# microsoft/fadtk

Measured on NVIDIA H100. Metric: audio_seconds_embedded_per_second, higher is better.
Workload: dtype f16

## Files before the change

fadtk_b200/csrc/fadtk_b200.cu:

```cuda
#include "../../include/fadtk_b200.h"

#include <cuda.h>
#include <cuda_runtime.h>
#include <cuda_fp16.h>
#include <cxxabi.h>
#include <algorithm>
#include <cmath>
#include <cstdio>
#include <cstdlib>
#include <cstring>
#include <memory>
#include <set>
#include <string>
#include <type_traits>
#include <utility>
#include <vector>

#include "conv_gemm.cuh"
#include "frontend.cuh"
#include "stats.cuh"
#include "frechet.cuh"
#include "clap.cuh"
#include "resample.cuh"
#include "whisper.cuh"
// ... 200 lines not shown
                 cudaLaunchAttribute* attrs, unsigned n_attrs, Args&&... args) {
    if (grid.x == 0 || grid.y == 0 || grid.z == 0) return 0;
    cudaLaunchConfig_t cfg = {};
    cfg.gridDim = grid;
    cfg.blockDim = block;
    cfg.dynamicSmemBytes = smem;
    cfg.stream = st;
    cfg.attrs = attrs;
    cfg.numAttrs = n_attrs;
    cudaError_t e = cudaLaunchKernelEx(&cfg, kernel, std::forward<Args>(args)...);
    const cudaError_t last = cudaGetLastError();
    if (e == cudaSuccess) e = last;
    if (e != cudaSuccess) return fail(kernel_name((const void*)kernel) + ": " + cudaGetErrorString(e));
    h->launches++;
    return 0;
}
template <typename... Params, typename... Args>
int launch(fad_handle* h, void (*kernel)(Params...), dim3 grid, dim3 block, size_t smem, cudaStream_t st, Args&&... args) {
    return launch_attrs(h, kernel, grid, block, smem, st, nullptr, 0, std::forward<Args>(args)...);
}

template <int WMODE> struct Gemm {
    static constexpr int kStages = WMODE ? 3 : 4;
    static constexpr uint32_t kSmem = fad::conv_gemm_smem_bytes<128, kStages, WMODE>();
    static_assert(kSmem <= 227 * 1024, "over the per-CTA shared-memory limit");
    static constexpr auto kernel = fad::conv_gemm_kernel<128, kStages, WMODE>;
};

cudaLaunchAttribute cta_pair() {
    cudaLaunchAttribute attr = {};
    attr.id = cudaLaunchAttributeClusterDimension;
    attr.val.clusterDim.x = fad::kClusterCtas; attr.val.clusterDim.y = 1; attr.val.clusterDim.z = 1;
    return attr;
}

template <int WMODE>
int setup_gemm(fad_handle* h) {
    CK(cudaFuncSetAttribute(Gemm<WMODE>::kernel, cudaFuncAttributeMaxDynamicSharedMemorySize, (int)Gemm<WMODE>::kSmem));
    cudaLaunchAttribute attr = cta_pair();
    cudaLaunchConfig_t cfg = {};
    cfg.gridDim = dim3(fad::kClusterCtas * (unsigned)h->num_sms);
    cfg.blockDim = dim3(fad::kConvGemmThreads);
    cfg.dynamicSmemBytes = Gemm<WMODE>::kSmem;
    cfg.attrs = &attr;
    cfg.numAttrs = 1;
    CK(cudaOccupancyMaxActiveClusters(&h->gemm_clusters[WMODE], Gemm<WMODE>::kernel, &cfg));
    if (h->gemm_clusters[WMODE] <= 0) return fail("conv_gemm_kernel: no CTA pair fits on the device");
    return 0;
}

template <int WMODE>
int launch_conv_gemm(fad_handle* h, const CUtensorMap& mx, const CUtensorMap& mw, const fad::ConvGemmParams& p, cudaStream_t st) {
    const int units = (p.img_groups * p.tiles_h * p.tiles_w + 1) / 2 * p.n_tiles;
    cudaLaunchAttribute attr = cta_pair();
    return launch_attrs(h, Gemm<WMODE>::kernel, dim3(fad::kClusterCtas * (unsigned)std::min(units, h->gemm_clusters[WMODE])),
                        dim3(fad::kConvGemmThreads), Gemm<WMODE>::kSmem, st, &attr, 1, mx, mw, p);
}

int encode_layer_maps(const LayerGeom& g, const void* x, long long nb_dim, const void* w,
                      CUtensorMap* mx, CUtensorMap* mw, int a_cols = 0, long long a_row_stride = 0) {
    const uint64_t ac = a_cols > 0 ? (uint64_t)a_cols : (uint64_t)g.Cin;
    const uint64_t xd[4] = {ac, (uint64_t)g.W, (uint64_t)g.H, (uint64_t)nb_dim};
    uint64_t xs[3] = {ac * 2, (uint64_t)g.W * ac * 2, (uint64_t)g.H * g.W * ac * 2};
    if (a_row_stride > 0) xs[0] = xs[1] = xs[2] = (uint64_t)a_row_stride * 2;
    const uint32_t xb[4] = {64, (uint32_t)g.box_w, (uint32_t)g.box_h, (uint32_t)g.box_n};
    if (encode_f16_map(mx, x, 4, xd, xs, xb)) return 1;
    const uint64_t K = (uint64_t)g.taps * g.Cin;
    const uint64_t rows_mul = g.split_w ? 2 : 1;
    const uint64_t wd[2] = {K, (uint64_t)g.Cout * rows_mul};
    const uint64_t ws[1] = {K * 2};
    const uint32_t wb[2] = {64, (uint32_t)(g.n_tile * rows_mul / fad::kClusterCtas)};
    return encode_f16_map(mw, w, 2, wd, ws, wb);
}

int launch_attention_wgmma(fad_handle* h, const __half* qkv, long long n_clips, int S, int d, int heads, __half* out, cudaStream_t st) {
    if (heads * 64 != d) return fail("attention_wgmma: head dimension must be 64");
    CUtensorMap map;
    const uint64_t dims[3] = {(uint64_t)3 * d, (uint64_t)S, (uint64_t)n_clips};
    const uint64_t strides[2] = {(uint64_t)3 * d * 2, (uint64_t)S * 3 * d * 2};
    const uint32_t box[3] = {64, 128, 1};
    if (encode_f16_map(&map, qkv, 3, dims, strides, box)) return 1;
    fad::AttnParams p;
    p.S = S; p.d = d; p.heads = heads; p.out = out;
    return launch(h, fad::attention_wgmma_kernel, dim3((S + 127) / 128, heads, (unsigned)n_clips), fad::kAtThreads, fad::kAtSmem,
                  st, map, p);
}

int run_layer(fad_handle* h, const LayerGeom& g, const CUtensorMap& mx, const CUtensorMap& mw, const void* w,
              int NB, const float* bias, void* out, float* out_f32, cudaStream_t st,
              float* resid = nullptr, int resid_C = 0, int resid_res = 0, int resid_shift = 0, int n_valid = 0) {
    fad::ConvGemmParams p;
    p.taps = g.taps; p.cblks = g.Cin / 64;
    p.box_w = g.box_w; p.box_h = g.box_h; p.box_n = g.box_n;
    p.tiles_w = g.W / g.box_w; p.tiles_h = g.H / g.box_h;
    p.img_groups = (NB + g.box_n - 1) / g.box_n;
    p.n_tiles = g.Cout / g.n_tile;
    p.H = g.H; p.W = g.W; p.NB = NB; p.Cout = g.Cout;
    p.n_valid = n_valid > 0 ? n_valid : g.Cout;
    p.ld_out = p.n_valid;
    p.relu = g.relu; p.pool = g.pool;
    p.bias = bias; p.out = reinterpret_cast<__half*>(out); p.out_f32 = out_f32;
    p.resid = resid; p.resid_C = resid_C; p.resid_res = resid_res; p.resid_shift = resid_shift;
    p.lo_adds = g.split_w == 1 && h->zero_lo.count(w) == 0;
    if (g.split_w) return launch_conv_gemm<1>(h, mx, mw, p, st);
    return launch_conv_gemm<0>(h, mx, mw, p, st);
}

__global__ void wlo_absmax_kernel(const __half* __restrict__ w, long long n_tiles, long long K, unsigned int* __restrict__ out) {
    float m = 0.f;
    const long long total = n_tiles * 128 * K;
    for (long long e = blockIdx.x * (long long)blockDim.x + threadIdx.x; e < total; e += (long long)gridDim.x * blockDim.x) {
        const long long row = e / K, k = e - row * K;
        const long long t = row >> 7, j = row & 127;
        m = fmaxf(m, fabsf(__half2float(w[((t * 256 + 128 + j) * K) + k])));
    }
    for (int o = 16; o > 0; o >>= 1) m = fmaxf(m, __shfl_xor_sync(0xffffffffu, m, o));
    if ((threadIdx.x & 31) == 0) atomicMax(out, __float_as_uint(m));
}
int note_split_weights(fad_handle* h, const void* w, long long n_tiles, long long K, cudaStream_t st) {
    DeviceBuffer d_max;
    if (d_max.grow(4)) return 1;
    unsigned int mx = 0;
    const unsigned blocks = (unsigned)std::max<long long>(1, std::min<long long>((n_tiles * 128 * K + 255) / 256, (long long)h->num_sms * 16));
    CK(cudaMemsetAsync(d_max.get(), 0, 4, st));
    if (launch(h, wlo_absmax_kernel, blocks, 256, 0, st, reinterpret_cast<const __half*>(w), n_tiles, K, d_max.get<unsigned int>()))
        return 1;
    CK(cudaMemcpyAsync(&mx, d_max.get(), 4, cudaMemcpyDeviceToHost, st));
    CK(cudaStreamSynchronize(st));
    if (mx == 0) h->zero_lo.insert(w); else h->zero_lo.erase(w);
    return 0;
}

int upload_split(fad_handle* h, std::vector<DeviceBuffer>& mem, __half** dst, const void* src, size_t n, size_t k) {
    if (upload(mem, dst, src, 2 * n * k * 2)) return 1;
    return note_split_weights(h, *dst, (long long)(n / 128), (long long)k, 0);
}

struct VggLayer { int H, W, Cin, Cout, taps, relu, pool; };
const VggLayer kVgg[8] = {
    {48, 32, 64, 128, 9, 1, 1},
    {24, 16, 128, 256, 9, 1, 0},
    {24, 16, 256, 256, 9, 1, 1},
    {12, 8, 256, 512, 9, 1, 0},
    {12, 8, 512, 512, 9, 1, 1},
    {1, 1, 12288, 4096, 1, 1, 0},
    {1, 1, 4096, 4096, 1, 1, 0},
    {1, 1, 4096, 128, 1, 0, 0},
};
const size_t kActElems[8] = {48 * 32 * 64, 24 * 16 * 128, 24 * 16 * 256, 12 * 8 * 256,
                             12 * 8 * 512, 6 * 4 * 512, 4096, 4096};

struct VggState {
    std::vector<DeviceBuffer> mem;
    float *conv1_w = nullptr, *conv1_b = nullptr;
    __half* w[8] = {};
    float* b[8] = {};
    float* logmel = nullptr;
    __half* act[8] = {};
    CUtensorMap map_x[8], map_w[8];
    LayerGeom geom[8];
};

void build_frontend_tables(std::vector<double>& tw, std::vector<double>& hann,
                           std::vector<double>& melw, std::vector<int>& mstart, std::vector<int>& mcount) {
    const double PI = 3.14159265358979323846;
    tw.resize(512); hann.resize(fad::kWin);
    for (int k = 0; k < 256; ++k) {
        tw[2 * k] = std::cos(-2.0 * PI * k / 512.0);
        tw[2 * k + 1] = std::sin(-2.0 * PI * k / 512.0);
    }
    for (int n = 0; n < fad::kWin; ++n) hann[n] = 0.5 - 0.5 * std::cos(2.0 * PI / fad::kWin * n);
    auto mel = [](double f) { return 1127.0 * std::log(1.0 + f / 700.0); };
    std::vector<double> bins(fad::kBins), edges(fad::kMel + 2);
    for (int i = 0; i < fad::kBins; ++i) bins[i] = mel(8000.0 * i / (fad::kBins - 1));
    const double lo = mel(125.0), hi = mel(7500.0);
    for (int i = 0; i < fad::kMel + 2; ++i) edges[i] = lo + (hi - lo) * i / (fad::kMel + 1);
    melw.assign(fad::kMel * fad::kMelMaxTaps, 0.0);
    mstart.assign(fad::kMel, 0); mcount.assign(fad::kMel, 0);
    for (int b = 0; b < fad::kMel; ++b) {
        const double l = edges[b], c = edges[b + 1], u = edges[b + 2];
        int first = -1, cnt = 0;
        for (int i = 1; i < fad::kBins; ++i) {
            const double w = std::fmax(0.0, std::fmin((bins[i] - l) / (c - l), (u - bins[i]) / (u - c)));
            if (w > 0.0) {
                if (first < 0) first = i;
                const int off = i - first;
                if (off < fad::kMelMaxTaps) { melw[b * fad::kMelMaxTaps + off] = w; cnt = off + 1; }
            }
        }
        mstart[b] = first < 0 ? 0 : first;
        mcount[b] = cnt;
    }
}

size_t prof_begin(fad_handle* h, cudaStream_t st) {
    if (!h->prof_on) return 0;
    if (h->ev_used == h->ev_pool.size()) { cudaEvent_t e; cudaEventCreate(&e); h->ev_pool.push_back(e); }
    cudaEventRecord(h->ev_pool[h->ev_used], st);
    return h->ev_used++;
}
void prof_end(fad_handle* h, int cat, size_t e0, cudaStream_t st) {
    if (!h->prof_on) return;
    const size_t e1 = prof_begin(h, st);
    h->spans.push_back({cat, e0, e1});
}

template <typename In>
int launch_stats_dmma(fad_handle* h, const In* E, long long n_rows, int d, const __half* shift, double* acc, cudaStream_t st) {
    constexpr bool kProf = sizeof(In) == 2;
    if (d <= 0 || d % 64 != 0) return fail("d must be a positive multiple of 64");
    fad::StatsDmmaParams p;
    p.n_rows = n_rows; p.d = d; p.n_tiles = d / fad::kSdTile;
    p.n_pairs = p.n_tiles * (p.n_tiles + 1) / 2;
    const long long stages = (n_rows + fad::kSdRows - 1) / fad::kSdRows;
    long long want = (4LL * h->num_sms + p.n_pairs - 1) / p.n_pairs;
    if (want < 1) want = 1;
    long long per = (stages + want - 1) / want;
    if (per < 4) per = 4;
    p.n_splits = (int)((stages + per - 1) / per);
    p.rows_per_split = per * fad::kSdRows;
    p.shift = shift;
    const size_t jobs = (size_t)p.n_pairs * p.n_splits;
    if (h->ws_tiles.grow(jobs * fad::kSdTile * fad::kSdTile * 8)) return 1;
    if (h->ws_sums.grow((size_t)p.n_tiles * p.n_splits * fad::kSdTile * 8)) return 1;
    p.ws_tiles = h->ws_tiles.get<double>(); p.ws_sums = h->ws_sums.get<double>();
    size_t ev = kProf ? prof_begin(h, st) : 0;
    if (launch(h, fad::stats_dmma_kernel<In>, (unsigned)jobs, 256, 0, st, E, p)) return 1;
    if (kProf) { prof_end(h, FAD_PROF_STATS, ev, st); ev = prof_begin(h, st); }
    if (launch(h, fad::stats_dmma_reduce_kernel, dim3(p.n_pairs, fad::kSdTile * fad::kSdTile / 256), 256, 0, st, p, acc)) return 1;
    if (kProf) prof_end(h, FAD_PROF_STATS_REDUCE, ev, st);
    return 0;
}

}

extern "C" {

int fad_version(void) { return 1; }

int fad_profile_enable(fad_handle* h, int on) {
    if (!h) return fail("null handle");
    h->prof_on = on != 0;
    return 0;
}

int fad_profile_collect(fad_handle* h, double* ms_out, long long* count_out, int reset) {
    if (!h) return fail("null handle");
    CK(cudaSetDevice(h->device));
    CK(cudaDeviceSynchronize());
    for (const auto& sp : h->spans) {
        float ms = 0.f;
        if (cudaEventElapsedTime(&ms, h->ev_pool[sp.e0], h->ev_pool[sp.e1]) == cudaSuccess) {
            h->prof_ms[sp.cat] += ms; h->prof_count[sp.cat]++;
        }
    }
    h->spans.clear(); h->ev_used = 0;
    for (int i = 0; i < FAD_PROF_CATEGORIES; ++i) {
        if (ms_out) ms_out[i] = h->prof_ms[i];
        if (count_out) count_out[i] = h->prof_count[i];
        if (reset) { h->prof_ms[i] = 0.0; h->prof_count[i] = 0; }
    }
    return 0;
}
const char* fad_last_error(void) { return g_err.c_str(); }

int fad_create(int device, int max_examples, fad_handle** out) {
    if (!out) return fail("null out pointer");
    int count = 0;
    if (cudaGetDeviceCount(&count) != cudaSuccess || count == 0)
        return fail("no CUDA device: fadtk_b200 has no CPU fallback");
    if (device < 0 || device >= count) return fail("bad device index");
    CK(cudaSetDevice(device));
    cudaDeviceProp prop;
    CK(cudaGetDeviceProperties(&prop, device));
    if (prop.major != 9) return fail("fadtk_b200 kernels are built for sm_90a (Hopper H100) only");
    std::unique_ptr<fad_handle> h(new fad_handle());
    h->device = device;
    h->num_sms = prop.multiProcessorCount;
    h->max_examples = max_examples > 0 ? max_examples : 2048;

    std::vector<double> tw, hann, melw; std::vector<int> ms, mc;
    build_frontend_tables(tw, hann, melw, ms, mc);
    if (upload(h->mem, &h->d_twiddle, tw.data(), tw.size() * 8) || upload(h->mem, &h->d_hann, hann.data(), hann.size() * 8) ||
        upload(h->mem, &h->d_melw, melw.data(), melw.size() * 8) || upload(h->mem, &h->d_mel_start, ms.data(), ms.size() * 4) ||
        upload(h->mem, &h->d_mel_count, mc.data(), mc.size() * 4)) return 1;
    const auto smem = [](const void* kernel, size_t bytes) {
        return cudaFuncSetAttribute(kernel, cudaFuncAttributeMaxDynamicSharedMemorySize, (int)bytes);
    };
    CK(smem((const void*)fad::logmel_kernel<double>, fad::logmel_smem_bytes<double>()));
    CK(smem((const void*)fad::logmel_kernel<float>, fad::logmel_smem_bytes<float>()));
    CK(smem((const void*)fad::clap_logmel_kernel, fad::clap_logmel_smem_bytes()));
    CK(smem((const void*)fad::attention_wgmma_kernel, fad::kAtSmem));
    CK(smem((const void*)fad::clap_window_attention_kernel<24>, fad::att_smem_bytes(24, fad::kAttWarps, fad::kAttStages)));
    CK(smem((const void*)fad::clap_window_attention_kernel<32>, fad::att_smem_bytes(32, fad::kAttWarps, fad::kAttStages)));
    CK(smem((const void*)fad::kad_tile_kernel<0>, fad::kKadSmemBytes));
    CK(smem((const void*)fad::kad_tile_kernel<1>, fad::kKadSmemBytes));
    CK(smem((const void*)fad::kad_tile_kernel<2>, fad::kKadSmemBytes));
    CK(smem((const void*)fad::kad_perm_tile_kernel, fad::kPermSmemBytes));
    CK(smem((const void*)fad::prdc_tile_kernel<0>, fad::kPairSmemBytes));
    CK(smem((const void*)fad::prdc_tile_kernel<1>, fad::kPairSmemBytes));
    CK(smem((const void*)fad::prdc_tile_kernel<2>, fad::kPairSmemBytes));
    CK(smem((const void*)fad::prdc_tile_kernel<3>, fad::kPrdcSongSmemBytes));
    CK(smem((const void*)fad::prdc_tile_kernel<4>, fad::kPairSmemBytes));
    CK(smem((const void*)fad::prdc_tile_kernel<5>, fad::kPrdcNearestSmemBytes));
    CK(smem((const void*)fad::prdc_tile_kernel<6>, fad::kPairSmemBytes));
    if (setup_gemm<0>(h.get()) || setup_gemm<1>(h.get())) return 1;
    *out = h.release();
    return 0;
}

int fad_destroy(fad_handle* h) {
    if (!h) return 0;
    cudaSetDevice(h->device);
    fad_comm_destroy(h);
    delete h;
    return 0;
}

long long fad_launch_count(fad_handle* h) { return h ? h->launches : 0; }

int fad_vggish_load(fad_handle* h, const fad_vggish_weights* w) {
    if (!h || !w) return fail("null argument");
    const void* src[18] = {w->conv1_w_host, w->conv1_b_host,
                           w->conv_w_host[0], w->conv_w_host[1], w->conv_w_host[2], w->conv_w_host[3], w->conv_w_host[4],
                           w->fc_w_host[0], w->fc_w_host[1], w->fc_w_host[2],
                           w->conv_b_host[0], w->conv_b_host[1], w->conv_b_host[2], w->conv_b_host[3], w->conv_b_host[4],
                           w->fc_b_host[0], w->fc_b_host[1], w->fc_b_host[2]};
    if (check_tensors("fad_vggish_load", src, 18)) return 1;
    const void* const* wsrc = src + 2;
    const void* const* bsrc = src + 10;
    CK(cudaSetDevice(h->device));
    h->vgg.reset();
    auto vs = std::make_unique<VggState>();
    auto& m = vs->mem;
    if (upload(m, &vs->conv1_w, src[0], 64 * 9 * 4) || upload(m, &vs->conv1_b, src[1], 64 * 4)) return 1;
    for (int i = 0; i < 8; ++i) {
        const VggLayer& L = kVgg[i];
        const size_t mul = ((w->split_mask >> i) & 1) ? 2 : 1;
        if (upload(m, &vs->w[i], wsrc[i], mul * L.Cout * L.taps * L.Cin * 2) || upload(m, &vs->b[i], bsrc[i], (size_t)L.Cout * 4))
            return 1;
    }
    for (int i = 0; i < 8; ++i)
        if (((w->split_mask >> i) & 1) &&
            note_split_weights(h, vs->w[i], kVgg[i].Cout / 128, (long long)kVgg[i].taps * kVgg[i].Cin, 0)) return 1;
    const size_t B = (size_t)h->max_examples;
    if (alloc(m, &vs->logmel, B * 96 * 64 * 4)) return 1;
    for (int i = 0; i < 8; ++i)
        if (alloc(m, &vs->act[i], B * kActElems[i] * 2)) return 1;
    for (int i = 0; i < 8; ++i) {
        const VggLayer& L = kVgg[i];
        if (make_geom(vs->geom[i], L.H, L.W, L.Cin, L.Cout, L.taps, L.relu, L.pool, (w->split_mask >> i) & 1)) return 1;
        if (encode_layer_maps(vs->geom[i], vs->act[i], (long long)B, vs->w[i], &vs->map_x[i], &vs->map_w[i])) return 1;
    }
    h->vgg = std::move(vs);
    return 0;
}

long long fad_vggish_num_examples(long long n_samples) {
    if (n_samples < fad::kWin) return 0;
    const long long t = 1 + (n_samples - fad::kWin) / fad::kHop;
    if (t < fad::kExFrames) return 0;
    return 1 + (t - fad::kExFrames) / fad::kExFrames;
}

long long fad_vggish_plan(const long long* clip_offsets_host, long long n_clips,
                          long long* ex_start_host, long long capacity, long long* rows_per_clip_host) {
    long long n = 0;
    for (long long c = 0; c < n_clips; ++c) {
        const long long len = clip_offsets_host[c + 1] - clip_offsets_host[c];
        const long long k = fad_vggish_num_examples(len);
        if (rows_per_clip_host) rows_per_clip_host[c] = k;
        for (long long e = 0; e < k; ++e, ++n)
            if (ex_start_host && n < capacity)
                ex_start_host[n] = clip_offsets_host[c] + e * (long long)(fad::kExFrames * fad::kHop);
    }
    return n;
}

static int launch_logmel(fad_handle* h, const int16_t* pcm, const long long* ex_start, long long n,
                         float* out, int use_double, cudaStream_t st) {
    fad::FrontendTables tab{h->d_twiddle, h->d_hann, h->d_melw, h->d_mel_start, h->d_mel_count};
    const long long frames = n * fad::kExFrames;
    long long blocks = (frames + fad::kFeWarps - 1) / fad::kFeWarps;
    const long long cap = (long long)h->num_sms * 8;
    if (blocks > cap) blocks = cap;
    if (use_double)
        return launch(h, fad::logmel_kernel<double>, (int)blocks, fad::kFeWarps * 32, fad::logmel_smem_bytes<double>(), st,
                      pcm, ex_start, (int)n, tab, out);
    return launch(h, fad::logmel_kernel<float>, (int)blocks, fad::kFeWarps * 32, fad::logmel_smem_bytes<float>(), st,
                  pcm, ex_start, (int)n, tab, out);
}

int fad_vggish_logmel(fad_handle* h, const int16_t* pcm, const long long* ex_start,
                      long long n_examples, float* logmel_out, int use_double, void* stream) {
    if (!h) return fail("null handle");
    CK(cudaSetDevice(h->device));
    return launch_logmel(h, pcm, ex_start, n_examples, logmel_out, use_double, (cudaStream_t)stream);
}

int fad_vggish_forward(fad_handle* h, const int16_t* pcm, const long long* ex_start,
                       long long n_examples, void* emb_out_f16, void* stream) {
    if (!h) return fail("null handle");
    if (!h->vgg) return fail("fad_vggish_load has not been called");
    CK(cudaSetDevice(h->device));
    const VggState& vs = *h->vgg;
    cudaStream_t st = (cudaStream_t)stream;
    static const int fe_double = []() { const char* e = getenv("FADTK_FRONTEND_FP64"); return (e && e[0] == '1') ? 1 : 0; }();
    for (long long base = 0; base < n_examples; base += h->max_examples) {
        const int nb = (int)((n_examples - base) < h->max_examples ? (n_examples - base) : h->max_examples);
        size_t ev = prof_begin(h, st);
        if (launch_logmel(h, pcm, ex_start + base, nb, vs.logmel, fe_double, st)) return 1;
        prof_end(h, FAD_PROF_LOGMEL, ev, st);
        ev = prof_begin(h, st);
        if (launch(h, fad::conv1_kernel, dim3(6, nb), 256, 0, st, vs.logmel, vs.conv1_w, vs.conv1_b, vs.act[0])) return 1;
        prof_end(h, FAD_PROF_CONV1, ev, st);
        for (int i = 0; i < 8; ++i) {
            void* out = (i == 7) ? (void*)((__half*)emb_out_f16 + (size_t)base * 128) : (void*)vs.act[i + 1];
            ev = prof_begin(h, st);
            if (run_layer(h, vs.geom[i], vs.map_x[i], vs.map_w[i], vs.w[i], nb, vs.b[i], out, nullptr, st)) return 1;
            prof_end(h, FAD_PROF_LAYER0 + i, ev, st);
        }
    }
    return 0;
}

int fad_vggish_conv1(fad_handle* h, const float* logmel, long long n_examples, void* out_f16, void* stream) {
    if (!h) return fail("null handle");
    if (!h->vgg) return fail("fad_vggish_load has not been called");
    if (n_examples <= 0) return 0;
    CK(cudaSetDevice(h->device));
    return launch(h, fad::conv1_kernel, dim3(6, (unsigned)n_examples), 256, 0, (cudaStream_t)stream,
                  logmel, h->vgg->conv1_w, h->vgg->conv1_b, reinterpret_cast<__half*>(out_f16));
}

int fad_umma_layer(fad_handle* h, const void* x_f16, int NB, int H, int W, int Cin,
                   const void* w_f16, const float* bias, int Cout, int taps, int relu, int pool,
                   int split_w, void* out_f16, float* out_f32_or_null, void* stream) {
    if (!h) return fail("null handle");
    if (split_w != 0 && split_w != 1) return fail("fad_umma_layer: split_w must be 0 (fp16 weights) or 1 (fp16 hi/lo pair)");
    CK(cudaSetDevice(h->device));
    LayerGeom g;
    if (make_geom(g, H, W, Cin, Cout, taps, relu, pool, split_w)) return 1;
    if (pool && out_f32_or_null) return fail("fp32 copy is only available for un-pooled layers");
    if (g.split_w == 1 && note_split_weights(h, w_f16, Cout / 128, (long long)taps * Cin, (cudaStream_t)stream)) return 1;
    CUtensorMap mx, mw;
    if (encode_layer_maps(g, x_f16, NB, w_f16, &mx, &mw)) return 1;
    return run_layer(h, g, mx, mw, w_f16, NB, bias, out_f16, out_f32_or_null, (cudaStream_t)stream);
}

size_t fad_stats_acc_len(int d) { return 1 + 2 * (size_t)d + (size_t)d * d; }

int fad_stats_accumulate(fad_handle* h, const void* emb_f16, long long n_rows, int d,
                         const void* shift_f16, double* acc, int tensor_core, void* stream) {
    if (!h) return fail("null handle");
    if (tensor_core != 0 && tensor_core != 2) return fail("fad_stats_accumulate: tensor_core must be 0 (DMMA) or 2 (CUDA-core fp64)");
    if (n_rows <= 0) return 0;
    CK(cudaSetDevice(h->device));
    cudaStream_t st = (cudaStream_t)stream;
    const __half* E = reinterpret_cast<const __half*>(emb_f16);
    const __half* shift = reinterpret_cast<const __half*>(shift_f16);
    if (tensor_core == 0) return launch_stats_dmma(h, E, n_rows, d, shift, acc, st);
    if (d % 64 != 0) return fail("d must be a multiple of 64");
    dim3 grid((unsigned)((n_rows + fad::kSimtRows - 1) / fad::kSimtRows), d / 64, d / 64);
    return launch(h, fad::stats_simt_kernel, grid, 256, 0, st, E, n_rows, d, shift, acc);
}

int fad_file_means(fad_handle* h, const void* emb_f16, long long n_files, int rows_per_file, int d,
                   double* m64_out, double* m16_out, void* stream) {
    if (!h) return fail("null handle");
    if (n_files <= 0) return 0;
    if (rows_per_file <= 0 || d <= 0) return fail("bad shape");
    CK(cudaSetDevice(h->device));
    long long blocks = (n_files * d + 255) / 256;
    if (blocks > (long long)h->num_sms * 16) blocks = (long long)h->num_sms * 16;
    return launch(h, fad::file_means_kernel, (unsigned)blocks, 256, 0, (cudaStream_t)stream,
                  reinterpret_cast<const __half*>(emb_f16), n_files, rows_per_file, d, m64_out, m16_out);
}

int fad_stats_accumulate_f64(fad_handle* h, const double* rows, long long n_rows, int d, double* acc, void* stream) {
    if (!h) return fail("null handle");
    if (n_rows <= 0) return 0;
    CK(cudaSetDevice(h->device));
    return launch_stats_dmma(h, rows, n_rows, d, nullptr, acc, (cudaStream_t)stream);
}

int fad_stats_finalize_mirrored(fad_handle* h, const double* acc, const double* acc_means64, const double* acc_means16,
                                const void* shift_f16, int rows_per_file, int d, double* mu_out, double* cov_out, void* stream) {
    if (!h) return fail("null handle");
    CK(cudaSetDevice(h->device));
    static const int keep = [] { const char* e = getenv("FADTK_SINGLE_FRAME_FILES"); return (e && std::string(e) == "keep") ? 1 : 0; }();
    const size_t total = (size_t)d * d;
    unsigned blocks = (unsigned)((total + 255) / 256);
    if (blocks > (unsigned)h->num_sms * 8) blocks = h->num_sms * 8;
    return launch(h, fad::stats_finalize_mirrored_kernel, blocks, 256, 0, (cudaStream_t)stream,
                  acc, acc_means64, acc_means16, reinterpret_cast<const __half*>(shift_f16), rows_per_file, d, keep, mu_out, cov_out);
}

int fad_stats_accumulate_gather(fad_handle* h, const void* emb_f16, long long n_src_rows,
                                const long long* idx, long long n_idx, int d,
                                const void* shift_f16, double* acc, void* stream) {
    if (!h) return fail("null handle");
    (void)n_src_rows;
    if (n_idx <= 0) return 0;
    if (d % 8 != 0) return fail("d must be a multiple of 8");
    CK(cudaSetDevice(h->device));
    if (h->gather_buf.grow((size_t)n_idx * d * 2)) return 1;
    __half* rows = h->gather_buf.get<__half>();
    const long long vecs = n_idx * (d / 8);
    long long blocks = (vecs + 255) / 256;
    if (blocks > (long long)h->num_sms * 16) blocks = (long long)h->num_sms * 16;
    if (launch(h, fad::gather_rows_kernel, (unsigned)blocks, 256, 0, (cudaStream_t)stream,
               reinterpret_cast<const __half*>(emb_f16), idx, n_idx, d, rows)) return 1;
    return launch_stats_dmma(h, rows, n_idx, d, reinterpret_cast<const __half*>(shift_f16), acc, (cudaStream_t)stream);
}

int fad_stats_finalize(fad_handle* h, const double* acc, const void* shift_f16, int d,
                       double* mu_out, double* cov_out, void* stream) {
    if (!h) return fail("null handle");
    CK(cudaSetDevice(h->device));
    const size_t total = (size_t)d * d;
    unsigned blocks = (unsigned)((total + 255) / 256);
    if (blocks > (unsigned)h->num_sms * 8) blocks = h->num_sms * 8;
    return launch(h, fad::stats_finalize_kernel, blocks, 256, 0, (cudaStream_t)stream,
                  acc, reinterpret_cast<const __half*>(shift_f16), d, mu_out, cov_out);
}

extern "C" int fad_attention(fad_handle* h, const void* qkv_f16, long long n_clips, int S, int d, void* out_f16, int legacy, void* stream) {
    if (!h || !qkv_f16 || !out_f16) return fail("null argument");
    if (d % 64 != 0 || S <= 0 || n_clips <= 0) return fail("bad shape");
    CK(cudaSetDevice(h->device));
    cudaStream_t st = (cudaStream_t)stream;
    if (!legacy) return launch_attention_wgmma(h, reinterpret_cast<const __half*>(qkv_f16), n_clips, S, d, d / 64, reinterpret_cast<__half*>(out_f16), st);
    return launch(h, fad::whisper_flash_attention_kernel, dim3((S + 63) / 64, d / 64, (unsigned)n_clips), 128, 0, st,
                  reinterpret_cast<const __half*>(qkv_f16), S, d, reinterpret_cast<__half*>(out_f16), nullptr, nullptr);
}


#include <dlfcn.h>
namespace {
struct NcclId { char bytes[128]; };
struct NcclApi {
    int (*GetUniqueId)(NcclId*) = nullptr;
    int (*CommInitRank)(void**, int, NcclId, int) = nullptr;
    int (*AllReduce)(const void*, void*, size_t, int, int, void*, cudaStream_t) = nullptr;
    int (*CommDestroy)(void*) = nullptr;
    int (*CommCount)(void*, int*) = nullptr;
    int (*CommUserRank)(void*, int*) = nullptr;
    const char* (*GetErrorString)(int) = nullptr;
    bool ok = false;
    std::string why;
};
NcclApi& nccl_api() {
    static NcclApi api = [] {
        NcclApi a;
        const char* env = getenv("FADTK_NCCL_LIB");
        const char* names[] = {env, "libnccl.so.2", "libnccl.so"};
        void* lib = nullptr;
        for (const char* n : names) {
            if (!n || !*n) continue;
            lib = dlopen(n, RTLD_NOW | RTLD_GLOBAL);
            if (lib) break;
        }
        if (!lib) { a.why = "libnccl.so.2 not found (set FADTK_NCCL_LIB)"; return a; }
        a.GetUniqueId = reinterpret_cast<decltype(a.GetUniqueId)>(dlsym(lib, "ncclGetUniqueId"));
        a.CommInitRank = reinterpret_cast<decltype(a.CommInitRank)>(dlsym(lib, "ncclCommInitRank"));
        a.AllReduce = reinterpret_cast<decltype(a.AllReduce)>(dlsym(lib, "ncclAllReduce"));
        a.CommDestroy = reinterpret_cast<decltype(a.CommDestroy)>(dlsym(lib, "ncclCommDestroy"));
        a.CommCount = reinterpret_cast<decltype(a.CommCount)>(dlsym(lib, "ncclCommCount"));
        a.CommUserRank = reinterpret_cast<decltype(a.CommUserRank)>(dlsym(lib, "ncclCommUserRank"));
        a.GetErrorString = reinterpret_cast<decltype(a.GetErrorString)>(dlsym(lib, "ncclGetErrorString"));
        a.ok = a.GetUniqueId && a.CommInitRank && a.AllReduce && a.CommDestroy && a.CommCount && a.CommUserRank &&
               a.GetErrorString;
        if (!a.ok) a.why = "NCCL library lacks an expected symbol";
        return a;
    }();
    return api;
}
int nccl_fail(const char* what, int rc) {
    return fail(std::string(what) + ": " + (nccl_api().GetErrorString ? nccl_api().GetErrorString(rc) : "NCCL error"));
}
}

extern "C" {
int fad_comm_unique_id(void* id_out_host) {
    if (!id_out_host) return fail("null argument");
// ... 267 lines not shown
```

fadtk_b200/csrc/frontend.cuh:

```cuda
#pragma once
#include <cuda_fp16.h>
#include <stdint.h>

namespace fad {

constexpr int kWin = 400, kHop = 160, kFft = 512, kBins = 257, kMel = 64, kExFrames = 96;
constexpr int kMelMaxTaps = 24;
constexpr int kFeWarps = 8;

struct FrontendTables {
    const double* twiddle;
    const double* hann;
    const double* mel_w;
    const int* mel_start;
    const int* mel_count;
};

template <typename T> struct Cx { T re, im; };

template <typename T>
__host__ __device__ constexpr size_t logmel_smem_bytes() {
    return sizeof(T) * (size_t)(kFeWarps * (2 * 256 + 260) + 2 * 256 + kWin + kMel * kMelMaxTaps)
         + sizeof(int) * 2 * kMel;
}

template <typename T> __device__ __forceinline__ Cx<T> cmul(Cx<T> a, Cx<T> b) {
    return {a.re * b.re - a.im * b.im, a.re * b.im + a.im * b.re};
}
template <typename T> __device__ __forceinline__ Cx<T> cadd(Cx<T> a, Cx<T> b) { return {a.re + b.re, a.im + b.im}; }
template <typename T> __device__ __forceinline__ Cx<T> csub(Cx<T> a, Cx<T> b) { return {a.re - b.re, a.im - b.im}; }
template <typename T> __device__ __forceinline__ Cx<T> mul_neg_i(Cx<T> a) { return {a.im, -a.re}; }

template <typename T> __device__ __forceinline__ void fft8(Cx<T> (&a)[8]) {
    const T c = (T)0.70710678118654752440;
    Cx<T> b0 = cadd(a[0], a[4]), b4 = csub(a[0], a[4]);
    Cx<T> b1 = cadd(a[1], a[5]), t1 = csub(a[1], a[5]);
    Cx<T> b2 = cadd(a[2], a[6]), b6 = mul_neg_i(csub(a[2], a[6]));
    Cx<T> b3 = cadd(a[3], a[7]), t3 = csub(a[3], a[7]);
    Cx<T> b5 = {c * (t1.re + t1.im), c * (t1.im - t1.re)};
    Cx<T> b7 = {c * (t3.im - t3.re), -c * (t3.re + t3.im)};
    Cx<T> q0 = cadd(b0, b2), q1 = cadd(b1, b3), q2 = csub(b0, b2), q3 = mul_neg_i(csub(b1, b3));
    a[0] = cadd(q0, q1); a[4] = csub(q0, q1); a[2] = cadd(q2, q3); a[6] = csub(q2, q3);
    Cx<T> r0 = cadd(b4, b6), r1 = cadd(b5, b7), r2 = csub(b4, b6), r3 = mul_neg_i(csub(b5, b7));
    a[1] = cadd(r0, r1); a[5] = csub(r0, r1); a[3] = cadd(r2, r3); a[7] = csub(r2, r3);
}

__device__ __forceinline__ float shfl_xor_t(float v, int m) { return __shfl_xor_sync(0xffffffffu, v, m); }
__device__ __forceinline__ double shfl_xor_t(double v, int m) { return __shfl_xor_sync(0xffffffffu, v, m); }

template <typename T>
__global__ void __launch_bounds__(kFeWarps * 32)
logmel_kernel(const int16_t* __restrict__ pcm, const long long* __restrict__ ex_start,
              int n_examples, FrontendTables tab, float* __restrict__ out)
{
    extern __shared__ __align__(16) unsigned char fe_smem[];
    T* sm = reinterpret_cast<T*>(fe_smem);
    Cx<T>* tw = reinterpret_cast<Cx<T>*>(sm);
    T* hann = sm + 512;
    T* melw = hann + kWin;
    T* wbuf = melw + kMel * kMelMaxTaps;
    int* mstart = reinterpret_cast<int*>(wbuf + kFeWarps * (512 + 260));
    int* mcount = mstart + kMel;

    for (int i = threadIdx.x; i < 256; i += blockDim.x) {
        tw[i].re = (T)tab.twiddle[2 * i]; tw[i].im = (T)tab.twiddle[2 * i + 1];
    }
    for (int i = threadIdx.x; i < kWin; i += blockDim.x) hann[i] = (T)tab.hann[i];
    for (int i = threadIdx.x; i < kMel * kMelMaxTaps; i += blockDim.x) melw[i] = (T)tab.mel_w[i];
    for (int i = threadIdx.x; i < kMel; i += blockDim.x) { mstart[i] = tab.mel_start[i]; mcount[i] = tab.mel_count[i]; }
    __syncthreads();

    const int warp = threadIdx.x >> 5, lane = threadIdx.x & 31;
    Cx<T>* z = reinterpret_cast<Cx<T>*>(wbuf + warp * (512 + 260));
    T* mag = wbuf + warp * (512 + 260) + 512;

    T hw[7][2];
#pragma unroll
    for (int n1 = 0; n1 < 7; ++n1) {
        const int n = 32 * n1 + lane;
        hw[n1][0] = n < kWin / 2 ? hann[2 * n] * (T)(1.0 / 32768.0) : (T)0;
        hw[n1][1] = n < kWin / 2 ? hann[2 * n + 1] * (T)(1.0 / 32768.0) : (T)0;
    }
    Cx<T> tw1[8];
#pragma unroll
    for (int k1 = 0; k1 < 8; ++k1) {
        const int m = 2 * lane * k1;
        const Cx<T> w = tw[m & 255];
        tw1[k1] = (m & 256) ? Cx<T>{-w.re, -w.im} : w;
    }
    Cx<T> tw2[5];
#pragma unroll
    for (int s = 0; s < 5; ++s) {
        const int h = 16 >> s;
        tw2[s] = tw[(lane & (h - 1)) * (256 / h)];
    }
    const int rev = __brev((unsigned)lane) >> 27;

    const long long total = (long long)n_examples * kExFrames;
    for (long long g = (long long)blockIdx.x * kFeWarps + warp; g < total;
         g += (long long)gridDim.x * kFeWarps) {
        const int e = (int)(g / kExFrames), f = (int)(g % kExFrames);
        const int16_t* src = pcm + ex_start[e] + (long long)f * kHop;

        Cx<T> a[8];
#pragma unroll
        for (int n1 = 0; n1 < 7; ++n1) {
            const int n = 32 * n1 + lane;
            if (n < kWin / 2) {
                a[n1].re = (T)src[2 * n] * hw[n1][0];
                a[n1].im = (T)src[2 * n + 1] * hw[n1][1];
            } else { a[n1].re = 0; a[n1].im = 0; }
        }
        a[7].re = 0; a[7].im = 0;
        fft8(a);
#pragma unroll
        for (int k1 = 1; k1 < 8; ++k1) a[k1] = cmul(a[k1], tw1[k1]);
#pragma unroll
        for (int s = 0; s < 5; ++s) {
            const int h = 16 >> s;
            const bool upper = (lane & h) != 0;
#pragma unroll
            for (int r = 0; r < 8; ++r) {
                Cx<T> p = {shfl_xor_t(a[r].re, h), shfl_xor_t(a[r].im, h)};
                a[r] = upper ? cmul(csub(p, a[r]), tw2[s]) : cadd(a[r], p);
            }
        }
#pragma unroll
        for (int k1 = 0; k1 < 8; ++k1) z[k1 + 8 * rev] = a[k1];
        __syncwarp();
        for (int k = lane; k <= 128; k += 32) {
            const Cx<T> x = z[k], y = z[(256 - k) & 255];
            const T er = (T)0.5 * (x.re + y.re), ei = (T)0.5 * (x.im - y.im);
            const T orr = (T)0.5 * (x.im + y.im), oi = (T)-0.5 * (x.re - y.re);
            const Cx<T> w = tw[k & 255];
            const T pr = orr * w.re - oi * w.im, pi = orr * w.im + oi * w.re;
            const T xr = er + pr, xi = ei + pi, yr = er - pr, yi = ei - pi;
            mag[k] = sqrt(xr * xr + xi * xi);
            mag[256 - k] = sqrt(yr * yr + yi * yi);
        }
        __syncwarp();
        float* dst = out + g * kMel;
#pragma unroll
        for (int hsel = 0; hsel < 2; ++hsel) {
            const int b = hsel ? 63 - lane : lane;
            const int st = mstart[b], cnt = mcount[b];
            T acc = 0;
            for (int i = 0; i < cnt; ++i) acc += mag[st + i] * melw[b * kMelMaxTaps + i];
            dst[b] = (float)log(acc + (T)0.01);
        }
        __syncwarp();
    }
}

__device__ __forceinline__ void mma_m16n8k16(float (&c)[4], uint32_t a0, uint32_t a1, uint32_t a2, uint32_t a3,
                                             uint32_t b0, uint32_t b1) {
    asm volatile("mma.sync.aligned.m16n8k16.row.col.f32.f16.f16.f32 {%0,%1,%2,%3}, {%4,%5,%6,%7}, {%8,%9}, {%0,%1,%2,%3};"
                 : "+f"(c[0]), "+f"(c[1]), "+f"(c[2]), "+f"(c[3])
                 : "r"(a0), "r"(a1), "r"(a2), "r"(a3), "r"(b0), "r"(b1));
}

__global__ void __launch_bounds__(256)
conv1_kernel(const float* __restrict__ logmel , const float* __restrict__ w ,
             const float* __restrict__ bias, __half* __restrict__ out )
{
    __shared__ float tile[18][68];
    const int e = blockIdx.y, strip = blockIdx.x;
    const int row0 = strip * 16 - 1;
    const float* src = logmel + (size_t)e * 96 * 64;
    for (int i = threadIdx.x; i < 18 * 66; i += 256) {
        const int r = i / 66, c = i % 66;
        const int gr = row0 + r, gc = c - 1;
        tile[r][c] = (gr >= 0 && gr < 96 && gc >= 0 && gc < 64) ? src[gr * 64 + gc] : 0.0f;
    }
    const int lane = threadIdx.x & 31, warp = threadIdx.x >> 5;
    float w0[9], w1[9];
#pragma unroll
    for (int i = 0; i < 9; ++i) { w0[i] = w[(2 * lane) * 9 + i]; w1[i] = w[(2 * lane + 1) * 9 + i]; }
    const float b0 = bias[2 * lane], b1 = bias[2 * lane + 1];
    __syncthreads();

    const int py = warp;
#pragma unroll 2
    for (int px = 0; px < 32; ++px) {
        float patch[4][4];
#pragma unroll
        for (int r = 0; r < 4; ++r)
#pragma unroll
            for (int c = 0; c < 4; ++c) patch[r][c] = tile[2 * py + r][2 * px + c];
        float m0 = -3.0e38f, m1 = -3.0e38f;
#pragma unroll
        for (int dy = 0; dy < 2; ++dy)
#pragma unroll
            for (int dx = 0; dx < 2; ++dx) {
                float a0 = 0.f, a1 = 0.f;
#pragma unroll
                for (int kh = 0; kh < 3; ++kh)
#pragma unroll
                    for (int kw = 0; kw < 3; ++kw) {
                        const float x = patch[dy + kh][dx + kw];
                        a0 = fmaf(w0[kh * 3 + kw], x, a0);
                        a1 = fmaf(w1[kh * 3 + kw], x, a1);
                    }
                m0 = fmaxf(m0, a0); m1 = fmaxf(m1, a1);
            }
        m0 = fmaxf(m0 + b0, 0.f); m1 = fmaxf(m1 + b1, 0.f);
        const size_t pix = ((size_t)e * 48 + strip * 8 + py) * 32 + px;
        *reinterpret_cast<__half2*>(out + pix * 64 + 2 * lane) = __floats2half2_rn(m0, m1);
    }
}

}
```

Before: 181,300.

## Rewrite VGGish conv1 as split-fp16 tensor-core MMA and tweak logmel smem layout

Result: faster. 184,900 (median of 6 runs) (+2.0%).

```diff
diff --git a/fadtk_b200/csrc/fadtk_b200.cu b/fadtk_b200/csrc/fadtk_b200.cu
--- a/fadtk_b200/csrc/fadtk_b200.cu
+++ b/fadtk_b200/csrc/fadtk_b200.cu
@@ -376,7 +376,8 @@
 
 struct VggState {
     std::vector<DeviceBuffer> mem;
-    float *conv1_w = nullptr, *conv1_b = nullptr;
+    __half* conv1_w = nullptr;
+    float* conv1_b = nullptr;
     __half* w[8] = {};
     float* b[8] = {};
     float* logmel = nullptr;
@@ -513,6 +514,7 @@
     };
     CK(smem((const void*)fad::logmel_kernel<double>, fad::logmel_smem_bytes<double>()));
     CK(smem((const void*)fad::logmel_kernel<float>, fad::logmel_smem_bytes<float>()));
+    CK(smem((const void*)fad::conv1_kernel, fad::kConv1Smem));
     CK(smem((const void*)fad::clap_logmel_kernel, fad::clap_logmel_smem_bytes()));
     CK(smem((const void*)fad::attention_wgmma_kernel, fad::kAtSmem));
     CK(smem((const void*)fad::clap_window_attention_kernel<24>, fad::att_smem_bytes(24, fad::kAttWarps, fad::kAttStages)));
@@ -557,7 +559,9 @@
     h->vgg.reset();
     auto vs = std::make_unique<VggState>();
     auto& m = vs->mem;
-    if (upload(m, &vs->conv1_w, src[0], 64 * 9 * 4) || upload(m, &vs->conv1_b, src[1], 64 * 4)) return 1;
+    std::vector<__half> conv1_wb(64 * fad::kConv1K);
+    fad::conv1_pack_weights(static_cast<const float*>(src[0]), conv1_wb.data());
+    if (upload(m, &vs->conv1_w, conv1_wb.data(), conv1_wb.size() * 2) || upload(m, &vs->conv1_b, src[1], 64 * 4)) return 1;
     for (int i = 0; i < 8; ++i) {
         const VggLayer& L = kVgg[i];
         const size_t mul = ((w->split_mask >> i) & 1) ? 2 : 1;
@@ -636,7 +640,8 @@
         if (launch_logmel(h, pcm, ex_start + base, nb, vs.logmel, fe_double, st)) return 1;
         prof_end(h, FAD_PROF_LOGMEL, ev, st);
         ev = prof_begin(h, st);
-        if (launch(h, fad::conv1_kernel, dim3(6, nb), 256, 0, st, vs.logmel, vs.conv1_w, vs.conv1_b, vs.act[0])) return 1;
+        if (launch(h, fad::conv1_kernel, nb, 256, fad::kConv1Smem, st, vs.logmel, reinterpret_cast<const uint4*>(vs.conv1_w),
+                   vs.conv1_b, vs.act[0])) return 1;
         prof_end(h, FAD_PROF_CONV1, ev, st);
         for (int i = 0; i < 8; ++i) {
             void* out = (i == 7) ? (void*)((__half*)emb_out_f16 + (size_t)base * 128) : (void*)vs.act[i + 1];
@@ -652,9 +657,11 @@
     if (!h) return fail("null handle");
     if (!h->vgg) return fail("fad_vggish_load has not been called");
     if (n_examples <= 0) return 0;
-    CK(cudaSetDevice(h->device));
-    return launch(h, fad::conv1_kernel, dim3(6, (unsigned)n_examples), 256, 0, (cudaStream_t)stream,
-                  logmel, h->vgg->conv1_w, h->vgg->conv1_b, reinterpret_cast<__half*>(out_f16));
+    if (((uintptr_t)logmel | (uintptr_t)out_f16) % 16 != 0)
+        return fail("fad_vggish_conv1: logmel and out must be 16-byte aligned (the kernel moves 16-B vectors)");
+    CK(cudaSetDevice(h->device));
+    return launch(h, fad::conv1_kernel, (unsigned)n_examples, 256, fad::kConv1Smem, (cudaStream_t)stream, logmel,
+                  reinterpret_cast<const uint4*>(h->vgg->conv1_w), h->vgg->conv1_b, reinterpret_cast<__half*>(out_f16));
 }
 
 int fad_umma_layer(fad_handle* h, const void* x_f16, int NB, int H, int W, int Cin,
diff --git a/fadtk_b200/csrc/frontend.cuh b/fadtk_b200/csrc/frontend.cuh
--- a/fadtk_b200/csrc/frontend.cuh
+++ b/fadtk_b200/csrc/frontend.cuh
@@ -47,6 +47,11 @@
 
 __device__ __forceinline__ float shfl_xor_t(float v, int m) { return __shfl_xor_sync(0xffffffffu, v, m); }
 __device__ __forceinline__ double shfl_xor_t(double v, int m) { return __shfl_xor_sync(0xffffffffu, v, m); }
+
+__device__ __forceinline__ int zslot(int k) {
+    const int r = (k & 7) | (k & 8);
+    return (r << 4) | ((k >> 4) ^ r);
+}
 
 template <typename T>
 __global__ void __launch_bounds__(kFeWarps * 32)
@@ -66,7 +71,8 @@
         tw[i].re = (T)tab.twiddle[2 * i]; tw[i].im = (T)tab.twiddle[2 * i + 1];
     }
     for (int i = threadIdx.x; i < kWin; i += blockDim.x) hann[i] = (T)tab.hann[i];
-    for (int i = threadIdx.x; i < kMel * kMelMaxTaps; i += blockDim.x) melw[i] = (T)tab.mel_w[i];
+    for (int i = threadIdx.x; i < kMel * kMelMaxTaps; i += blockDim.x)
+        melw[(i % kMelMaxTaps) * kMel + i / kMelMaxTaps] = (T)tab.mel_w[i];
     for (int i = threadIdx.x; i < kMel; i += blockDim.x) { mstart[i] = tab.mel_start[i]; mcount[i] = tab.mel_count[i]; }
     __syncthreads();
 
@@ -126,10 +132,10 @@
             }
         }
 #pragma unroll
-        for (int k1 = 0; k1 < 8; ++k1) z[k1 + 8 * rev] = a[k1];
+        for (int k1 = 0; k1 < 8; ++k1) z[zslot(k1 + 8 * rev)] = a[k1];
         __syncwarp();
         for (int k = lane; k <= 128; k += 32) {
-            const Cx<T> x = z[k], y = z[(256 - k) & 255];
+            const Cx<T> x = z[zslot(k)], y = z[zslot((256 - k) & 255)];
             const T er = (T)0.5 * (x.re + y.re), ei = (T)0.5 * (x.im - y.im);
             const T orr = (T)0.5 * (x.im + y.im), oi = (T)-0.5 * (x.re - y.re);
             const Cx<T> w = tw[k & 255];
@@ -145,7 +151,7 @@
             const int b = hsel ? 63 - lane : lane;
             const int st = mstart[b], cnt = mcount[b];
             T acc = 0;
-            for (int i = 0; i < cnt; ++i) acc += mag[st + i] * melw[b * kMelMaxTaps + i];
+            for (int i = 0; i < cnt; ++i) acc += mag[st + i] * melw[i * kMel + b];
             dst[b] = (float)log(acc + (T)0.01);
         }
         __syncwarp();
@@ -159,54 +165,141 @@
                  : "r"(a0), "r"(a1), "r"(a2), "r"(a3), "r"(b0), "r"(b1));
 }
 
-__global__ void __launch_bounds__(256)
-conv1_kernel(const float* __restrict__ logmel , const float* __restrict__ w ,
+constexpr int kConv1K = 32;
+inline void conv1_pack_weights(const float* w , __half* wb ) {
+    auto split = [](float wf, bool lo) {
+        const __half wh = __float2half_rn(wf);
+        return lo ? __float2half_rn(wf - __half2float(wh)) : wh;
+    };
+    for (int j = 0; j < 8; ++j)
+        for (int n = 0; n < 8; ++n) {
+            const float* wc = w + (16 * (n >> 1) + 2 * j + (n & 1)) * 9;
+            for (int k = 0; k < kConv1K; ++k) {
+                const int q = k >> 1, e = k & 1;
+                __half v = __float2half_rn(0.f);
+                if (q < 9) {
+                    v = split(wc[q], false);
+                } else if (q < 15) {
+                    const int kh = (q - 9) >> 1, kw = 2 * ((q - 9) & 1) + e;
+                    if (kw < 3) v = split(wc[kh * 3 + kw], true);
+                }
+                wb[(((8 * j + n) * 4 + (q & 3)) * 4 + (q >> 2)) * 2 + e] = v;
+            }
+        }
+}
+
+constexpr int kC1Row = 67, kC1Rows = 98, kC1H = kC1Rows * kC1Row + 5;
+constexpr int kC1StPix = 9;
+constexpr size_t kConv1Smem = (size_t)(kC1H + kC1Rows * kC1Row) * 4 + 256 * 16 + 32 * 8 + 8 * 16 * kC1StPix * 16;
+
+__global__ void __launch_bounds__(256, 2)
+conv1_kernel(const float* __restrict__ logmel , const uint4* __restrict__ wb ,
              const float* __restrict__ bias, __half* __restrict__ out )
 {
-    __shared__ float tile[18][68];
-    const int e = blockIdx.y, strip = blockIdx.x;
-    const int row0 = strip * 16 - 1;
-    const float* src = logmel + (size_t)e * 96 * 64;
-    for (int i = threadIdx.x; i < 18 * 66; i += 256) {
-        const int r = i / 66, c = i % 66;
-        const int gr = row0 + r, gc = c - 1;
-        tile[r][c] = (gr >= 0 && gr < 96 && gc >= 0 && gc < 64) ? src[gr * 64 + gc] : 0.0f;
-    }
+    extern __shared__ __align__(16) unsigned char c1_smem[];
+    uint4* wsm = reinterpret_cast<uint4*>(c1_smem);
+    float2* bsm = reinterpret_cast<float2*>(wsm + 256);
+    uint32_t* tile = reinterpret_cast<uint32_t*>(reinterpret_cast<uint4*>(bsm + 32) + 8 * 16 * kC1StPix);
+    __half* tile_h = reinterpret_cast<__half*>(tile);
+    const int e = blockIdx.x;
     const int lane = threadIdx.x & 31, warp = threadIdx.x >> 5;
-    float w0[9], w1[9];
-#pragma unroll
-    for (int i = 0; i < 9; ++i) { w0[i] = w[(2 * lane) * 9 + i]; w1[i] = w[(2 * lane + 1) * 9 + i]; }
-    const float b0 = bias[2 * lane], b1 = bias[2 * lane + 1];
+    const int g = lane >> 2, t = lane & 3;
+    uint4* st = reinterpret_cast<uint4*>(bsm + 32) + warp * 16 * kC1StPix;
+
+    for (int i = threadIdx.x; i < 4 * 66; i += 256) {
+        const int r = (i / 66) & 1 ? kC1Rows - 1 : 0;
+        tile[(i < 2 * 66 ? 0 : kC1H) + r * kC1Row + i % 66] = 0u;
+    }
+    for (int r = 1 + threadIdx.x; r < kC1Rows - 1; r += 256) {
+        tile[r * kC1Row] = 0u; tile[r * kC1Row + 65] = 0u; tile[kC1H + r * kC1Row + 65] = 0u;
+        tile_h[2 * (kC1H + r * kC1Row)] = __float2half_rn(0.f);
+        tile_h[2 * (kC1H + r * kC1Row + 64) + 1] = __float2half_rn(0.f);
+    }
+    const float4* src = reinterpret_cast<const float4*>(logmel + (size_t)e * 96 * 64);
+    float4 v[6];
+#pragma unroll
+    for (int it = 0; it < 6; ++it) v[it] = src[threadIdx.x + 256 * it];
+#pragma unroll
+    for (int it = 0; it < 6; ++it) {
+        const int i = threadIdx.x + 256 * it;
+        const int w0 = ((i >> 4) + 1) * kC1Row + (i & 15) * 4 + 1;
+        const float x[4] = {v[it].x, v[it].y, v[it].z, v[it].w};
+#pragma unroll
+        for (int q = 0; q < 4; ++q) {
+            const __half xh = __float2half_rn(x[q]);
+            const __half2 il = __halves2half2(xh, __float2half_rn(x[q] - __half2float(xh)));
+            tile[w0 + q] = *reinterpret_cast<const uint32_t*>(&il);
+            tile_h[2 * (kC1H + w0 + q)] = xh;
+            tile_h[2 * (kC1H + w0 + q - 1) + 1] = xh;
+        }
+    }
+    wsm[threadIdx.x] = wb[threadIdx.x];
+    if (threadIdx.x < 32) bsm[threadIdx.x] = reinterpret_cast<const float2*>(bias)[threadIdx.x];
+
+    auto aoff = [](int q) -> int {
+        if (q < 9) return (q / 3) * kC1Row + q % 3;
+        if (q < 15) return kC1H + ((q - 9) >> 1) * kC1Row + 2 * ((q - 9) & 1);
+        return 0;
+    };
+    int off[4];
+#pragma unroll
+    for (int i = 0; i < 4; ++i) off[i] = aoff(4 * i + t);
     __syncthreads();
 
-    const int py = warp;
-#pragma unroll 2
-    for (int px = 0; px < 32; ++px) {
-        float patch[4][4];
-#pragma unroll
-        for (int r = 0; r < 4; ++r)
-#pragma unroll
-            for (int c = 0; c < 4; ++c) patch[r][c] = tile[2 * py + r][2 * px + c];
-        float m0 = -3.0e38f, m1 = -3.0e38f;
-#pragma unroll
-        for (int dy = 0; dy < 2; ++dy)
-#pragma unroll
-            for (int dx = 0; dx < 2; ++dx) {
-                float a0 = 0.f, a1 = 0.f;
-#pragma unroll
-                for (int kh = 0; kh < 3; ++kh)
-#pragma unroll
-                    for (int kw = 0; kw < 3; ++kw) {
-                        const float x = patch[dy + kh][dx + kw];
-                        a0 = fmaf(w0[kh * 3 + kw], x, a0);
-                        a1 = fmaf(w1[kh * 3 + kw], x, a1);
-                    }
-                m0 = fmaxf(m0, a0); m1 = fmaxf(m1, a1);
+#pragma unroll 1
+    for (int u = warp; u < 96; u += 8) {
+        const int py = u >> 1, px0 = (u & 1) * 16;
+        uint32_t a[4][2][4];
+#pragma unroll
+        for (int sub = 0; sub < 4; ++sub) {
+            const uint32_t* p0 = tile + (2 * py + (sub >> 1)) * kC1Row + 2 * (px0 + g) + (sub & 1);
+            const uint32_t* p1 = p0 + 16;
+#pragma unroll
+            for (int s = 0; s < 2; ++s) {
+                a[sub][s][0] = p0[off[2 * s]]; a[sub][s][1] = p1[off[2 * s]];
+                a[sub][s][2] = p0[off[2 * s + 1]]; a[sub][s][3] = p1[off[2 * s + 1]];
             }
-        m0 = fmaxf(m0 + b0, 0.f); m1 = fmaxf(m1 + b1, 0.f);
-        const size_t pix = ((size_t)e * 48 + strip * 8 + py) * 32 + px;
-        *reinterpret_cast<__half2*>(out + pix * 64 + 2 * lane) = __floats2half2_rn(m0, m1);
-    }
-}
-
-}
+        }
+#pragma unroll 1
+        for (int jh = 0; jh < 2; ++jh) {
+          uint4 bf[4];
+          float mx[4][4];
+#pragma unroll
+          for (int jj = 0; jj < 4; ++jj) {
+            bf[jj] = wsm[(8 * (4 * jh + jj) + g) * 4 + t];
+            mx[jj][0] = mx[jj][1] = mx[jj][2] = mx[jj][3] = -3.0e38f;
+          }
+#pragma unroll
+          for (int sub = 0; sub < 4; ++sub)
+#pragma unroll
+            for (int jj = 0; jj < 4; ++jj) {
+                float acc[4] = {0.f, 0.f, 0.f, 0.f};
+                mma_m16n8k16(acc, a[sub][0][0], a[sub][0][1], a[sub][0][2], a[sub][0][3], bf[jj].x, bf[jj].y);
+                mma_m16n8k16(acc, a[sub][1][0], a[sub][1][1], a[sub][1][2], a[sub][1][3], bf[jj].z, bf[jj].w);
+#pragma unroll
+                for (int q = 0; q < 4; ++q) mx[jj][q] = fmaxf(mx[jj][q], acc[q]);
+            }
+          uint32_t h0[4], h1[4];
+#pragma unroll
+          for (int jj = 0; jj < 4; ++jj) {
+            const float2 b = bsm[8 * t + 4 * jh + jj];
+            const __half2 q0 = __floats2half2_rn(fmaxf(mx[jj][0] + b.x, 0.f), fmaxf(mx[jj][1] + b.y, 0.f));
+            const __half2 q1 = __floats2half2_rn(fmaxf(mx[jj][2] + b.x, 0.f), fmaxf(mx[jj][3] + b.y, 0.f));
+            h0[jj] = *reinterpret_cast<const uint32_t*>(&q0);
+            h1[jj] = *reinterpret_cast<const uint32_t*>(&q1);
+          }
+          st[g * kC1StPix + 2 * t + jh] = make_uint4(h0[0], h0[1], h0[2], h0[3]);
+          st[(g + 8) * kC1StPix + 2 * t + jh] = make_uint4(h1[0], h1[1], h1[2], h1[3]);
+        }
+        __syncwarp();
+        uint4* o = reinterpret_cast<uint4*>(out + (((size_t)e * 48 + py) * 32 + px0) * 64);
+#pragma unroll
+        for (int k = 0; k < 4; ++k) {
+            const int c = lane + 32 * k;
+            o[c] = st[(c >> 3) * kC1StPix + (c & 7)];
+        }
+        __syncwarp();
+    }
+}
+
+}
```
